# pinellolab/GRAFIMO

Hardware: AMD Instinct MI355X
Metric: scored haplotype k-mers/sec (higher is better)
Workload: dtype int32

## Files before the change

grafimo_amd/csrc/gfm_score_kernels.hpp:

```cpp
#pragma once

#include "gfm_common.hpp"

namespace {

constexpr int kWave = 64;
constexpr int kThreads = 1024;
constexpr int kWavesPerWG = kThreads / kWave;
constexpr unsigned kPoison = 0xFFFFu;
constexpr int kMaxLdsBytes = 160 * 1024;
constexpr int kWGsPerCU = 1;
constexpr int kReserveCUs = 4;
constexpr int kHitQueue = 64;

constexpr int kWorkspaces = GFM_WORKSPACE_RING;
constexpr int kCtlSlots = 2 * GFM_WORKSPACE_RING;
constexpr int kCtlAhead = GFM_WORKSPACE_RING;
struct HitCtl {
    unsigned long long mid[kCtlSlots];
    unsigned long long snap[kCtlSlots];
};
constexpr int kResidPerWG = kWavesPerWG * kHitQueue;

__device__ inline void hitq_push(long long *hitq, int &qn, bool hit, long long entry, int lane,
                                 const unsigned long long *hit_count, unsigned long long *mid,
                                 long long *hit_rows, long long hit_cap)
{
    const unsigned long long mask = __builtin_amdgcn_ballot_w64(hit);
    if (!mask) return;
    const int nh = __popcll(mask);
    if (qn + nh > kHitQueue) {
        unsigned long long base = 0;
        if (lane == 0) base = (hit_count ? *hit_count : 0ull) + atomicAdd(mid, (unsigned long long)qn);
        base = __shfl(base, 0);
        for (int i = lane; i < qn; i += kWave)
            if ((long long)(base + i) < hit_cap) hit_rows[base + i] = hitq[i];
        qn = 0;
    }
    if (hit) hitq[qn + __popcll(mask & ((1ull << lane) - 1ull))] = entry;
    qn += nh;
}

template <int WAVES>
__device__ inline void hitq_finish(const long long *hitq, int qn, int *wq_n ,
                                   int wave, int lane, int tid, long long *resid, int *resid_n)
{
    if (lane == 0) wq_n[wave] = qn;
    __syncthreads();
    int base = 0, tot = 0;
#pragma unroll
    for (int w = 0; w < WAVES; ++w) {
        if (w < wave) base += wq_n[w];
        tot += wq_n[w];
    }
    long long *slab = resid + (size_t)blockIdx.x * kResidPerWG;
    for (int i = lane; i < qn; i += kWave) slab[base + i] = hitq[i];
    if (tid == 0) resid_n[blockIdx.x] = tot;
}

constexpr int kSpillCopies = 16;

struct MotifArgs {
    const uint16_t *tab;
    int lo, nb, min_val;
    int use_hist;
    int spill_lo;
    int spill_n;
    unsigned *spill;
    int cutoff;
    int slot;
    int *scores;
    unsigned *partials;
    long long *hit_rows;
    long long hit_cap;
    const unsigned long long *hit_count;
    HitCtl *ctl;
    long long *resid;
    int *resid_n;
};
template <int MM> struct ScoreArgs {
    MotifArgs m[MM];
    int store_through;
};

typedef __attribute__((address_space(3))) const unsigned lds_cu32;
typedef __attribute__((address_space(3))) const uint16_t lds_cu16;
typedef __attribute__((address_space(3))) const unsigned long long lds_cu64;
__device__ inline unsigned lds_offset(const void *p)
{
    return (unsigned)(size_t)(__attribute__((address_space(3))) const char *)p;
}

constexpr int kSlabsPerGroup = 16;
constexpr int kPostJobs = 3;
struct PostJob {
    const unsigned *partials;
    unsigned long long *hist64;
    unsigned *spill;
    const long long *resid;
    const int *resid_n;
    HitCtl *ctl;
    long long *hit_rows;
    unsigned long long *hit_count;
    long long hit_cap;
    int nslabs, nb, lo, min_val, bin_blocks, hist_blocks, spill_lo, spill_n, spill_blocks, hit_slabs, par, total;
};
struct PostJobs { PostJob j[kPostJobs]; };

__device__ inline void
post_body(const unsigned *__restrict__ partials, int nslabs, int nb, int lo, int min_val,
          unsigned long long *__restrict__ hist64, int bin_blocks, int hist_blocks,
          unsigned *__restrict__ spill, int spill_lo, int spill_n, int spill_blocks,
          const long long *__restrict__ resid, const int *__restrict__ resid_n, int hit_slabs,
          HitCtl *__restrict__ ctl, int par, long long *__restrict__ hit_rows, long long hit_cap,
          unsigned long long *__restrict__ hit_count)
{
    const int tid = threadIdx.x;
    if (blockIdx.x == 0 && tid == 0 && hit_slabs == 0 && ctl) ctl->mid[(par + kCtlAhead) % kCtlSlots] = 0ull;
    if ((int)blockIdx.x < hist_blocks) {
        const int bx = blockIdx.x % bin_blocks, by = blockIdx.x / bin_blocks;
        const int b = bx * 256 + tid;
        if (b > nb) return;
        const int g0 = by * kSlabsPerGroup;
        const int g1 = min(g0 + kSlabsPerGroup, nslabs);
        unsigned long long s = 0;
        const size_t stride = (size_t)(nb + 1);
#pragma unroll 8
        for (int g = g0; g < g1; ++g) s += __builtin_nontemporal_load(&partials[g * stride + b]);
        if (s) atomicAdd(&hist64[b == nb ? min_val : lo + b], s);
        return;
    }
    if ((int)blockIdx.x < hist_blocks + spill_blocks) {
        const int b = ((int)blockIdx.x - hist_blocks) * 256 + tid;
        if (b < spill_n) {
            unsigned long long v = 0;
#pragma unroll
            for (int c = 0; c < kSpillCopies; ++c) {
                const unsigned x = spill[(size_t)c * (size_t)spill_n + b];
                if (x) {
                    v += x;
                    spill[(size_t)c * (size_t)spill_n + b] = 0u;
                }
            }
            if (v) atomicAdd(&hist64[spill_lo + b], v);
        }
        return;
    }
    __shared__ int part[256];
    __shared__ int part_all[256];
    const int g = blockIdx.x - hist_blocks - spill_blocks;
    int s = 0, sa = 0;
    for (int k = tid; k < hit_slabs; k += 256) {
        const int v = resid_n[k];
        sa += v;
        if (k < g) s += v;
    }
    part[tid] = s;
    part_all[tid] = sa;
    __syncthreads();
    for (int d = 128; d > 0; d >>= 1) {
        if (tid < d) { part[tid] += part[tid + d]; part_all[tid] += part_all[tid + d]; }
        __syncthreads();
    }
    const unsigned long long start = ctl->snap[par] + ctl->mid[par];
    const unsigned long long base = start + (unsigned long long)part[0];
    const int cnt = resid_n[g];
    const long long *slab = resid + (size_t)g * kResidPerWG;
    for (int i = tid; i < cnt; i += 256)
        if ((long long)(base + i) < hit_cap) __builtin_nontemporal_store(__builtin_nontemporal_load(&slab[i]), &hit_rows[base + i]);
    if (g == 0 && tid == 0) {
        *hit_count = start + (unsigned long long)part_all[0];
        ctl->mid[(par + kCtlAhead) % kCtlSlots] = 0ull;
    }
}

__global__ void __launch_bounds__(256) post_kernel(const PostJobs jobs)
{
    const PostJob &q = jobs.j[blockIdx.y];
    if ((int)blockIdx.x >= q.total) return;
    post_body(q.partials, q.nslabs, q.nb, q.lo, q.min_val, q.hist64, q.bin_blocks, q.hist_blocks, q.spill, q.spill_lo,
              q.spill_n, q.spill_blocks, q.resid, q.resid_n, q.hit_slabs, q.ctl, q.par, q.hit_rows, q.hit_cap,
              q.hit_count);
}

constexpr int kSelThreads = 256;
__global__ void __launch_bounds__(kSelThreads)
select_hits_kernel(const int *__restrict__ scores, long long n, const int *__restrict__ cutoff_ptr,
                   long long row_base, long long *__restrict__ hit_rows, long long hit_cap,
                   const unsigned long long *__restrict__ hit_count, HitCtl *__restrict__ ctl,
                   int par, long long *__restrict__ resid, int *__restrict__ resid_n,
                   const unsigned long long *__restrict__ gate_count, long long gate_cap)
{
    __shared__ long long hq[kSelThreads / kWave][kHitQueue];
    __shared__ int wq_n[kSelThreads / kWave];
    const int cutoff = *cutoff_ptr;
    const int tid = threadIdx.x, lane = tid & 63, wave = tid >> 6;
    long long *hitq = hq[wave];
    int qn = 0;
    if (gate_count) {
        if ((long long)*gate_count <= gate_cap) {
            if (tid == 0) {
                resid_n[blockIdx.x] = 0;
                if (blockIdx.x == 0) ctl->snap[par] = hit_count ? *hit_count : 0ull;
            }
            return;
        }
        hit_count = nullptr;
    }
    if (blockIdx.x == 0 && tid == 0) ctl->snap[par] = hit_count ? *hit_count : 0ull;
    const long long nthreads = (long long)gridDim.x * blockDim.x;
    const long long n4 = (n + 3) >> 2;
    const long long iters = (n4 + nthreads - 1) / nthreads;
    const long long t0 = (long long)blockIdx.x * blockDim.x + tid;
    for (long long it = 0; it < iters; ++it) {
        const long long i = t0 + it * nthreads;
        int sc[4] = {INT32_MIN, INT32_MIN, INT32_MIN, INT32_MIN};
        if (i * 4 + 4 <= n) {
            const int4 v = reinterpret_cast<const int4 *>(scores)[i];
            sc[0] = v.x; sc[1] = v.y; sc[2] = v.z; sc[3] = v.w;
        } else {
            for (int j = 0; j < 4; ++j)
                if (i * 4 + j < n) sc[j] = scores[i * 4 + j];
        }
#pragma unroll
        for (int j = 0; j < 4; ++j)
            hitq_push(hitq, qn, sc[j] >= cutoff,
                      ((row_base + i * 4 + j) << GFM_HIT_SCORE_BITS) | (long long)sc[j], lane,
                      hit_count, &ctl->mid[par], hit_rows, hit_cap);
    }
    hitq_finish<kSelThreads / kWave>(hitq, qn, wq_n, wave, lane, tid, resid, resid_n);
}

constexpr int kFilterPerThread = 16;
constexpr int kFilterPerBlock = kSelThreads * kFilterPerThread;
__global__ void __launch_bounds__(kSelThreads)
filter_hits_kernel(const long long *__restrict__ cand, const unsigned long long *__restrict__ cand_count,
                   long long cand_cap, const int *__restrict__ cutoff_ptr, long long *__restrict__ hit_rows,
                   long long hit_cap, unsigned long long *__restrict__ hit_count)
{
    __shared__ int wave_tot[kSelThreads / kWave];
    __shared__ unsigned long long block_base;
    const int cutoff = *cutoff_ptr;
    const int tid = threadIdx.x, lane = tid & 63, wave = tid >> 6;
    const unsigned long long have = *cand_count;
    if ((long long)have > cand_cap) {
        if (blockIdx.x == 0 && tid == 0) *hit_count = have;
        return;
    }
    const long long n = (long long)have;
    const long long first = (long long)blockIdx.x * kFilterPerBlock;
    if (first >= n) return;
    long long e[kFilterPerThread];
    int mine = 0;
#pragma unroll
    for (int j = 0; j < kFilterPerThread; ++j) {
        const long long i = first + (long long)j * kSelThreads + tid;
        e[j] = i < n ? cand[i] : -1ll;
        const bool keep = i < n && (int)(e[j] & ((1ll << GFM_HIT_SCORE_BITS) - 1)) >= cutoff;
        if (!keep) e[j] = -1ll;
        mine += keep ? 1 : 0;
    }
    int incl = mine;
#pragma unroll
    for (int d = 1; d < kWave; d <<= 1) {
        const int v = __shfl_up(incl, d);
        if (lane >= d) incl += v;
    }
    if (lane == kWave - 1) wave_tot[wave] = incl;
    __syncthreads();
    int before = 0, total = 0;
#pragma unroll
    for (int w = 0; w < kSelThreads / kWave; ++w) {
        if (w < wave) before += wave_tot[w];
        total += wave_tot[w];
    }
    if (tid == 0) block_base = total ? atomicAdd(hit_count, (unsigned long long)total) : 0ull;
    __syncthreads();
    unsigned long long at = block_base + (unsigned long long)(before + incl - mine);
#pragma unroll
    for (int j = 0; j < kFilterPerThread; ++j)
        if (e[j] >= 0) {
// ... 7 lines not shown
```

grafimo_amd/csrc/gfm_stats_kernels.hpp:

```cpp
#pragma once

#include "gfm_common.hpp"

namespace {

struct DpJob {
    long long sm;
    long long cum;
    long long bg;
    int W, L, lo, hi;
    double *buf;
    double *pmf;
    double *ptable;
};

constexpr int kDpThreads = 1024;

__global__ void __launch_bounds__(kDpThreads)
pvalue_dp_kernel(const DpJob *__restrict__ jobs, const int *__restrict__ ints, const double *__restrict__ dbls)
{
    const DpJob job = jobs[blockIdx.x];
    const int W = job.W, L = job.L;
    const int *__restrict__ sm = ints + job.sm;
    const int *__restrict__ cum_lo = ints + job.cum;
// ... 128 lines not shown
    unsigned long long a = 0, t = 0;
    for (int b = tid; b < nblk; b += kQThreads) {
        const unsigned long long v = ws->blk_cnt[b];
        t += v;
        if (b > blk) a += v;
    }
    const unsigned long long n = block_sum_u64(t, sh) + ws->n_rows_N;
    const unsigned long long above_blocks = block_sum_u64(a, sh);
    const double nd = (double)n;
    const int j = lo + blk * kQThreads + tid;
    const bool ok = j <= hi;
    const unsigned long long h = ok ? hist[j] : 0ull;
    unsigned long long cs = h;
#pragma unroll
    for (int d = 1; d < kWave; d <<= 1) {
        const unsigned long long v = __shfl_down(cs, d);
        if (lane + d < kWave) cs += v;
    }
    if (lane == 0) sh[wave] = cs;
    __syncthreads();
    unsigned long long waves_above = 0;
#pragma unroll
    for (int w = 0; w < kQThreads / kWave; ++w)
        if (w > wave) waves_above += sh[w];
    const unsigned long long c_ge = cs + waves_above + above_blocks;
    const double raw = h ? ptable[j] / ((double)c_ge / nd) : INFINITY;
    if (ok) raw_out[j] = raw;
    double m = raw;
#pragma unroll
    for (int d = 32; d > 0; d >>= 1) m = fmin(m, __shfl_down(m, d));
    if (lane == 0) shm[wave] = m;
    __syncthreads();
    if (tid == 0) {
        double bm = INFINITY;
        for (int w = 0; w < kQThreads / kWave; ++w) bm = fmin(bm, shm[w]);
        ws->blk_min[blk] = bm;
    }
}

__device__ inline void
q_final_body(const unsigned long long *hist, const double *__restrict__ ptable, int L, int lo,
             int hi, int min_val, double threshold, int on_qvalue, const QWork *__restrict__ ws,
             double *qtable, int *__restrict__ cutoff_out, unsigned long long *__restrict__ nrows_out,
             unsigned long long *__restrict__ clear, int nblk)
{
    __shared__ unsigned long long sh[kQThreads / kWave];
    __shared__ double shm[kQThreads / kWave];
    __shared__ int first_s;
    const int tid = threadIdx.x, lane = tid & 63, wave = tid >> 6;
    const int blk = blockIdx.x;
    if (tid == 0) first_s = L;
    unsigned long long t = 0;
    double below = INFINITY, all = INFINITY;
    for (int b = tid; b < nblk; b += kQThreads) {
        t += ws->blk_cnt[b];
        const double v = ws->blk_min[b];
        all = fmin(all, v);
        if (b < blk) below = fmin(below, v);
    }
    const unsigned long long n_rows_N = ws->n_rows_N;
    const unsigned long long n = block_sum_u64(t, sh) + n_rows_N;
    const double nd = (double)n;
#pragma unroll
    for (int d = 32; d > 0; d >>= 1) {
        below = fmin(below, __shfl_down(below, d));
        all = fmin(all, __shfl_down(all, d));
    }
    __shared__ double shb[kQThreads / kWave], sha[kQThreads / kWave];
    if (lane == 0) { shb[wave] = below; sha[wave] = all; }
    __syncthreads();
    below = INFINITY; all = INFINITY;
#pragma unroll
    for (int w = 0; w < kQThreads / kWave; ++w) { below = fmin(below, shb[w]); all = fmin(all, sha[w]); }
    const double base = n_rows_N ? ptable[min_val] / (nd / nd) : INFINITY;
    const int j = lo + blk * kQThreads + tid;
    const bool ok = j <= hi;
    double ms = ok ? qtable[j] : INFINITY;
#pragma unroll
    for (int d = 1; d < kWave; d <<= 1) {
        const double v = __shfl_up(ms, d);
        if (lane >= d) ms = fmin(ms, v);
    }
    if (lane == kWave - 1) shm[wave] = ms;
    __syncthreads();
    double waves_below = INFINITY;
#pragma unroll
    for (int w = 0; w < kQThreads / kWave; ++w)
        if (w < wave) waves_below = fmin(waves_below, shm[w]);
    const double q = fmin(fmin(fmin(ms, waves_below), fmin(below, base)), 1.0);
    if (ok) {
        qtable[j] = q;
        const double val = on_qvalue ? q : ptable[j];
        if (val < threshold) atomicMin(&first_s, j);
        if (clear) clear[j] = 0ull;
    }
    const int gtid = blk * kQThreads + tid, gsz = nblk * kQThreads;
    const double q_above = fmin(fmin(base, all), 1.0);
    for (int jj = gtid; jj < lo; jj += gsz) qtable[jj] = fmin(base, 1.0);
    for (int jj = hi + 1 + gtid; jj < L; jj += gsz) qtable[jj] = q_above;
    __syncthreads();
    if (tid == 0) {
        if (cutoff_out && first_s < L) atomicMin(cutoff_out, first_s);
        if (blk == 0) {
            if (nrows_out) *nrows_out = n;
            const bool n_outside = min_val < lo || min_val > hi;
            if (clear && n_outside) clear[min_val] = 0ull;
        }
    }
}

constexpr int kQJobs = 8;
struct QJob {
    const unsigned long long *hist;
    const double *ptable;
    QWork *ws;
    double *qtable;
    int *cutoff;
    unsigned long long *nrows;
    unsigned long long *clear;
    int L, lo, hi, min_val, nblk;
};
struct QJobs {
    QJob j[kQJobs];
    double threshold;
    int on_qvalue;
};

__global__ void __launch_bounds__(kQThreads) q_count_kernel(const QJobs jobs)
{
    const QJob &q = jobs.j[blockIdx.y];
    if ((int)blockIdx.x >= q.nblk) return;
    q_count_body(q.hist, q.L, q.lo, q.hi, q.min_val, q.ws, q.cutoff);
}

__global__ void __launch_bounds__(kQThreads) q_raw_kernel(const QJobs jobs)
{
    const QJob &q = jobs.j[blockIdx.y];
    if ((int)blockIdx.x >= q.nblk) return;
    q_raw_body(q.hist, q.ptable, q.lo, q.hi, q.ws, q.qtable, q.nblk);
}

__global__ void __launch_bounds__(kQThreads) q_final_kernel(const QJobs jobs)
{
    const QJob &q = jobs.j[blockIdx.y];
    if ((int)blockIdx.x >= q.nblk) return;
    q_final_body(q.hist, q.ptable, q.L, q.lo, q.hi, q.min_val, jobs.threshold, jobs.on_qvalue, q.ws, q.qtable,
                 q.cutoff, q.nrows, q.clear, q.nblk);
}

constexpr int kQ1Threads = 512;
constexpr int kQ1K = 16;
constexpr int kQ1Bins = kQ1Threads * kQ1K;
constexpr int kQ1Waves = kQ1Threads / kWave;

__global__ void __launch_bounds__(kQ1Threads) q_table_kernel(const QJobs jobs)
{
    const QJob &q = jobs.j[blockIdx.x];
    const unsigned long long *hist = q.hist;
    const double *__restrict__ ptable = q.ptable;
    double *qtable = q.qtable;
    unsigned long long *clear = q.clear;
    const int L = q.L, lo = q.lo, hi = q.hi, min_val = q.min_val;
    __shared__ unsigned long long sh_cnt[kQ1Waves];
    __shared__ double sh_min[kQ1Waves];
    __shared__ unsigned long long sh_n_rows_N;
    __shared__ int first_s;
    const int tid = threadIdx.x, lane = tid & (kWave - 1), wave = tid >> 6;
    const int j0 = lo + tid * kQ1K;
    const bool n_outside = min_val < lo || min_val > hi;
    if (tid == 0) {
        sh_n_rows_N = n_outside ? hist[min_val] : 0ull;
        first_s = L;
    }
    unsigned long long c[kQ1K];
    double p[kQ1K];
    unsigned occ = 0;
#pragma unroll
    for (int k = 0; k < kQ1K; ++k) c[k] = j0 + k <= hi ? hist[j0 + k] : 0ull;
#pragma unroll
    for (int k = 0; k < kQ1K; ++k) p[k] = j0 + k <= hi ? ptable[j0 + k] : 0.0;
    const double p_min_val = ptable[min_val];
    unsigned long long run = 0;
#pragma unroll
    for (int k = kQ1K - 1; k >= 0; --k) {
        occ |= (c[k] != 0ull ? 1u : 0u) << k;
        run += c[k];
        c[k] = run;
    }
    unsigned long long cs = run;
#pragma unroll
    for (int d = 1; d < kWave; d <<= 1) {
        const unsigned long long v = __shfl_down(cs, d);
        if (lane + d < kWave) cs += v;
    }
    if (lane == 0) sh_cnt[wave] = cs;
    __syncthreads();
    unsigned long long above = cs - run, total = 0;
#pragma unroll
    for (int w = 0; w < kQ1Waves; ++w) {
        const unsigned long long v = sh_cnt[w];
        total += v;
        if (w > wave) above += v;
    }
    const unsigned long long n_rows_N = sh_n_rows_N;
    const unsigned long long n = total + n_rows_N;
    const double nd = (double)n;
    double r[kQ1K];
    double m = INFINITY;
    unsigned p_below = 0;
#pragma unroll
    for (int k = 0; k < kQ1K; ++k) {
        double raw = INFINITY;
        if ((occ >> k) & 1u) raw = p[k] / ((double)(c[k] + above) / nd);
        p_below |= (p[k] < jobs.threshold ? 1u : 0u) << k;
        m = fmin(m, raw);
        r[k] = m;
    }
    double ms = m;
#pragma unroll
    for (int d = 1; d < kWave; d <<= 1) {
        const double v = __shfl_up(ms, d);
        if (lane >= d) ms = fmin(ms, v);
    }
    if (lane == kWave - 1) sh_min[wave] = ms;
    double below = __shfl_up(ms, 1);
    if (lane == 0) below = INFINITY;
    __syncthreads();
    double all = INFINITY;
#pragma unroll
    for (int w = 0; w < kQ1Waves; ++w) {
        const double v = sh_min[w];
        all = fmin(all, v);
        if (w < wave) below = fmin(below, v);
    }
    const double base = n_rows_N ? p_min_val / (nd / nd) : INFINITY;
    below = fmin(below, base);
    int first = L;
#pragma unroll
    for (int k = kQ1K - 1; k >= 0; --k) {
        const int j = j0 + k;
        if (j <= hi) {
            const double qv = fmin(fmin(r[k], below), 1.0);
            qtable[j] = qv;
            if (jobs.on_qvalue ? qv < jobs.threshold : ((p_below >> k) & 1u) != 0) first = j;
            if (clear) clear[j] = 0ull;
        }
    }
    if (first < L) atomicMin(&first_s, first);
    const double q_above = fmin(fmin(base, all), 1.0);
    for (int jj = tid; jj < lo; jj += kQ1Threads) qtable[jj] = fmin(base, 1.0);
    for (int jj = hi + 1 + tid; jj < L; jj += kQ1Threads) qtable[jj] = q_above;
    __syncthreads();
    if (tid == 0) {
        if (q.cutoff) *q.cutoff = first_s;
        if (q.nrows) *q.nrows = n;
        if (clear && n_outside) clear[min_val] = 0ull;
    }
}

}
```

grafimo_amd/csrc/grafimo_hip.hip:

```cpp

#include <hip/hip_runtime.h>

#include <algorithm>
#include <atomic>
#include <cmath>
#include <cstdarg>
#include <cstdint>
#include <cstdio>
#include <cstdlib>
#include <cstring>
#include <new>
#include <string>
#include <vector>

#include "grafimo_hip.h"

#define GFM_API extern "C" __attribute__((visibility("default")))

#include "gfm_hit_sort.hpp"
#include "gfm_common.hpp"
#include "gfm_score_kernels.hpp"
#include "gfm_quad_launch.hpp"
#include "gfm_stats_kernels.hpp"

struct gfm_motif {
    int W = 0, L = 0, min_val = 0, scale = 1, ndw = 0;
    double offset = 0.0;
    int lo = 0, hi = 0, nb = 0;
    int hlo = 0, hnb = 0;
    int q_waves = kWavesPerWG;
    int part_nb = 0;
    struct Window { int bins, lo; double mass; };
    std::vector<Window> windows;
    int device = 0;
    int n_cu = 256;
    int max_slabs = 0;
    int sel_slabs = 0;
    int reserve_cus = kReserveCUs;
    size_t lds_bytes = 0;
    std::vector<int64_t> sm;
    double bg[4] = {0, 0, 0, 0};
    std::vector<double> h_ptable;
    unsigned char *d_slab = nullptr;
    uint16_t *d_tab = nullptr;
    unsigned *d_ftab = nullptr;
    double *d_pmf = nullptr;
    double *d_ptable = nullptr;
    unsigned *d_partials[kWorkspaces] = {};
    unsigned *d_spill[kWorkspaces] = {};
    long long *d_resid[kWorkspaces] = {};
    int *d_resid_n[kWorkspaces] = {};
    QWork *d_qwork = nullptr;
    double *d_qscratch = nullptr;
    hipStream_t q_stream[kQStreams] = {};
    int q_streams_used = 0;
    unsigned long long q_last_use[kQStreams] = {}, q_calls = 0;
    hipEvent_t ev_selected = nullptr;
    hipStream_t sel_last_stream = nullptr;
    bool sel_valid = false;
    HitCtl *d_ctl = nullptr;
    unsigned call_no = 0;
    hipStream_t last_st = nullptr, last_tail = nullptr;
    unsigned same_pair_run = 0;
    hipEvent_t ev_scored[kWorkspaces] = {};
    hipStream_t launch_st[2] = {};
    hipEvent_t launch_last[2] = {};
    hipEvent_t ev_join[kWorkspaces] = {};
    unsigned quiet = 0;
    bool overlap_on = true;
    unsigned long long overlapped = 0;
    hipEvent_t ev_posted[kWorkspaces] = {};
    bool posted_valid[kWorkspaces] = {};
    long long *d_sel_resid = nullptr;
    int *d_sel_resid_n = nullptr;
    HitCtl *d_sel_ctl = nullptr;
    unsigned sel_call_no = 0;
    std::vector<hipEvent_t> ev0, ev1;
    int ev_next = 0, ev_used = 0, ev_every = 1;
    unsigned ev_calls = 0;
    std::vector<hipEvent_t> tev0, tev1;
    int ev_last = -1;
    int tail_pending = -1;
    std::vector<int> tail_order;
};

namespace {

int ensure_device()
{
    int n = 0;
    hipError_t e = hipGetDeviceCount(&n);
    if (e != hipSuccess || n <= 0) {
        (void)hipGetLastError();
        return fail(GFM_ERR_NODEVICE, "no HIP device available (%s)",
                    e == hipSuccess ? "device count is 0" : hipGetErrorString(e));
    }
    return GFM_OK;
}

void cumulative_windows(const int64_t *sm, int W, std::vector<int> &lo, std::vector<int> &hi)
{
    lo.resize(W);
    hi.resize(W);
    long long l = 0, h = 0;
    for (int j = 0; j < W; ++j) {
        int64_t mn = sm[j], mx = sm[j];
        for (int nuc = 1; nuc < 4; ++nuc) {
            mn = std::min(mn, sm[nuc * W + j]);
            mx = std::max(mx, sm[nuc * W + j]);
        }
        l += mn;
        h += mx;
        lo[j] = (int)l;
        hi[j] = (int)h;
    }
}

int validate_matrix(const int64_t *sm, int W, int i)
{
    if (!sm) return fail(GFM_ERR_INVALID, "motif %d: score matrix is NULL", i);
    if (W < 1 || W > GFM_MAX_WIDTH)
        return fail(GFM_ERR_INVALID, "motif %d: motif width %d outside [1, %d]", i, W, GFM_MAX_WIDTH);
    for (int k = 0; k < 4 * W; ++k)
        if (sm[k] < 0 || sm[k] > kRange)
            return fail(GFM_ERR_INVALID, "motif %d: scaled score %lld outside [0, %d]", i, (long long)sm[k], kRange);
    return GFM_OK;
}

size_t align256(size_t bytes) { return (bytes + 255) & ~(size_t)255; }

struct DpPack {
    std::vector<DpJob> jobs;
    std::vector<int> ints;
    std::vector<double> dbls;

    DpJob &add(const int64_t *sm, int W, const double *bg)
    {
        std::vector<int> lo, hi;
        cumulative_windows(sm, W, lo, hi);
        DpJob j{};
        j.sm = (long long)ints.size();
        for (int i = 0; i < 4 * W; ++i) ints.push_back((int)sm[i]);
        j.cum = (long long)ints.size();
        ints.insert(ints.end(), lo.begin(), lo.end());
        ints.insert(ints.end(), hi.begin(), hi.end());
        j.bg = (long long)dbls.size();
        dbls.insert(dbls.end(), bg, bg + 4);
        j.W = W;
        j.L = kRange * W + 1;
        j.lo = lo[W - 1];
        j.hi = hi[W - 1];
        jobs.push_back(j);
        return jobs.back();
    }
    size_t ints_at() const { return align256(sizeof(DpJob) * jobs.size()); }
    size_t dbls_at() const { return ints_at() + align256(sizeof(int) * ints.size()); }
    size_t bytes() const { return dbls_at() + sizeof(double) * dbls.size(); }
    std::vector<unsigned char> image() const
    {
        std::vector<unsigned char> img(bytes(), 0);
        std::memcpy(img.data(), jobs.data(), sizeof(DpJob) * jobs.size());
        std::memcpy(img.data() + ints_at(), ints.data(), sizeof(int) * ints.size());
        std::memcpy(img.data() + dbls_at(), dbls.data(), sizeof(double) * dbls.size());
        return img;
    }
    int launch(const unsigned char *d, int n_dp, bool tails, hipStream_t st) const
    {
        const DpJob *d_jobs = reinterpret_cast<const DpJob *>(d);
        if (n_dp > 0) {
            hipLaunchKernelGGL(pvalue_dp_kernel, dim3((unsigned)n_dp), dim3(kDpThreads), 0, st, d_jobs,
                               reinterpret_cast<const int *>(d + ints_at()),
                               reinterpret_cast<const double *>(d + dbls_at()));
            HIP_TRY(hipGetLastError());
        }
        if (tails && !jobs.empty()) {
            hipLaunchKernelGGL(ptable_kernel, dim3((unsigned)jobs.size()), dim3(kScanThreads), 0, st, d_jobs);
            HIP_TRY(hipGetLastError());
        }
        return GFM_OK;
    }
};

int dispatch_quad(int W, int mm, gfm_motif *timer, const uint8_t *d_kmers, long long n, long long row_base,
                  const void *args, size_t lds, int nslabs, int waves, hipStream_t st, bool prepare_only,
                  hipEvent_t *done = nullptr)
{
    if (W < 1 || W > GFM_MAX_WIDTH) return fail(GFM_ERR_INVALID, "unsupported width %d", W);
    if (mm < 1 || mm > 3 || (mm > 1 && W > kQuadMaxBatchWidth))
        return fail(GFM_ERR_INVALID, "no kernel for %d motifs of width %d in one launch", mm, W);
    hipEvent_t e0 = nullptr, e1 = done ? *done : nullptr;
    if (!prepare_only && timer && !timer->ev0.empty() && (timer->ev_calls++ % (unsigned)timer->ev_every) == 0) {
        e0 = timer->ev0[timer->ev_next];
        e1 = timer->ev1[timer->ev_next];
        if (done) *done = e1;
        timer->ev_last = timer->ev_next;
        timer->ev_next = (timer->ev_next + 1) % (int)timer->ev0.size();
        timer->ev_used = std::min(timer->ev_used + 1, (int)timer->ev0.size());
    } else if (timer) {
        timer->ev_last = -1;
    }
    typedef int (*launch_fn)(int, const uint8_t *, long long, long long, const void *, size_t, int, int, void *, int,
                             void *, void *);
    static const launch_fn table[3][4] = {
        {gfm_quad_launch_g0_m1, gfm_quad_launch_g1_m1, gfm_quad_launch_g2_m1, gfm_quad_launch_g3_m1},
        {gfm_quad_launch_g0_m2, gfm_quad_launch_g1_m2, nullptr, nullptr},
        {gfm_quad_launch_g0_m3, gfm_quad_launch_g1_m3, nullptr, nullptr}};
    return table[mm - 1][(W - 1) / 16](W, d_kmers, n, row_base, args, lds, nslabs, waves, st, prepare_only ? 1 : 0, e0, e1);
}

constexpr long long kStoreThroughMaxBytes = 96ll << 20;
int score_store_through(long long n, int mm)
{
#ifdef GFM_LAB
    if (const char *e = std::getenv("GRAFIMO_STORE_POLICY")) {
        if (!std::strcmp(e, "through")) return 1;
        if (!std::strcmp(e, "stream")) return 0;
    }
#endif
    return n * 4ll * mm <= kStoreThroughMaxBytes ? 1 : 0;
}

size_t quad_fixed_lds(int W, int waves, int mm = 1)
{
    return (size_t)quad_tab_bytes(W, mm) + (size_t)waves * (size_t)quad_strip_stride(W, mm);
}

gfm_motif::Window best_window(gfm_motif *m, int bins)
{
    if (bins >= m->nb) return {m->nb, m->lo, 1.0};
    for (const auto &w : m->windows)
        if (w.bins == bins) return w;
    gfm_motif::Window best{bins, m->lo, -1.0};
    for (int a = m->lo; a + bins - 1 <= m->hi; ++a) {
        const int e = a + bins;
        const double mass = m->h_ptable[a] - (e < m->L ? m->h_ptable[e] : 0.0);
        if (mass > best.mass) { best.mass = mass; best.lo = a; }
    }
    m->windows.push_back(best);
    return best;
}

PostJob post_job(gfm_motif *m, const unsigned *partials, int hist_slabs, unsigned long long *d_hist,
                 int win_lo, int win_nb, unsigned *spill, const long long *resid, const int *resid_n, int hit_slabs,
                 HitCtl *ctl, int ctl_slot, long long *d_hit_rows, long long cap, unsigned long long *d_hit_count)
{
    PostJob q{};
    q.bin_blocks = (win_nb + 1 + 255) / 256;
    const int groups = (hist_slabs + kSlabsPerGroup - 1) / kSlabsPerGroup;
    q.hist_blocks = d_hist ? q.bin_blocks * groups : 0;
    q.spill_blocks = (d_hist && spill && win_nb < m->nb) ? (m->nb + 255) / 256 : 0;
    q.total = q.hist_blocks + q.spill_blocks + hit_slabs;
    q.partials = partials; q.hist64 = d_hist; q.spill = spill; q.resid = resid; q.resid_n = resid_n; q.ctl = ctl;
    q.hit_rows = d_hit_rows; q.hit_count = d_hit_count; q.hit_cap = cap;
    q.nslabs = hist_slabs; q.nb = win_nb; q.lo = win_lo; q.min_val = m->min_val;
    q.spill_lo = m->lo; q.spill_n = m->nb; q.hit_slabs = hit_slabs; q.par = ctl_slot;
    return q;
}

int launch_posts(const PostJob *jobs, int count, hipStream_t st)
{
    PostJobs all{};
    int live = 0, max_total = 0;
    for (int k = 0; k < count; ++k) {
        const PostJob &q = jobs[k];
        if (q.total == 0) {
            if (q.ctl)
                HIP_TRY(hipMemsetAsync(&q.ctl->mid[(q.par + kCtlAhead) % kCtlSlots], 0, sizeof(unsigned long long), st));
            continue;
        }
        all.j[live++] = q;
        max_total = std::max(max_total, q.total);
    }
    if (live == 0) return GFM_OK;
    hipLaunchKernelGGL(post_kernel, dim3((unsigned)max_total, (unsigned)live), dim3(256), 0, st, all);
    HIP_TRY(hipGetLastError());
    return GFM_OK;
}

int launch_post(gfm_motif *m, const unsigned *partials, int hist_slabs, unsigned long long *d_hist,
                int win_lo, int win_nb, unsigned *spill, const long long *resid, const int *resid_n, int hit_slabs, HitCtl *ctl, int ctl_slot,
                long long *d_hit_rows, long long cap, unsigned long long *d_hit_count, hipStream_t st)
{
    const PostJob q = post_job(m, partials, hist_slabs, d_hist, win_lo, win_nb, spill, resid, resid_n, hit_slabs, ctl,
                               ctl_slot, d_hit_rows, cap, d_hit_count);
    return launch_posts(&q, 1, st);
}

int join_launch_streams(gfm_motif *m, hipStream_t st)
{
    for (int i = 0; i < 2; ++i) {
        if (!m->launch_last[i]) continue;
        HIP_TRY(hipStreamWaitEvent(st, m->launch_last[i], 0));
        m->launch_last[i] = nullptr;
    }
    return GFM_OK;
}

__global__ void launch_stream_warm_kernel() {}

int ensure_launch_streams(gfm_motif *m)
{
    for (int i = 0; i < 2; ++i) {
        if (m->launch_st[i]) continue;
        HIP_TRY(hipStreamCreateWithFlags(&m->launch_st[i], hipStreamNonBlocking));
        hipLaunchKernelGGL(launch_stream_warm_kernel, dim3(1), dim3(kWave), 0, m->launch_st[i]);
        HIP_TRY(hipGetLastError());
    }
    for (int i = 0; i < kWorkspaces; ++i)
        if (!m->ev_join[i]) HIP_TRY(hipEventCreateWithFlags(&m->ev_join[i], hipEventDisableTiming));
    return GFM_OK;
}

int caller_stream_idle(gfm_motif *m, hipStream_t st, bool *idle)
{
    *idle = false;
    if (m->quiet) {
        --m->quiet;
        return GFM_OK;
    }
    const hipError_t q = hipStreamQuery(st);
    if (q != hipSuccess) {
        (void)hipGetLastError();
        if (q != hipErrorNotReady) HIP_TRY(q);
        m->quiet = 3;
        return GFM_OK;
    }
    *idle = true;
    return GFM_OK;
}

void fill_motif_args(MotifArgs &a, gfm_motif *m, int ws, int slot, int use_hist, int win_lo, int win_nb,
                     int cutoff,
                     int *d_scores, long long *d_hit_rows, long long cap,
                     const unsigned long long *d_hit_count_or_null)
{
    a.tab = m->d_tab;
    a.lo = win_lo;
    a.nb = win_nb;
    a.min_val = m->min_val;
    a.use_hist = use_hist;
    a.spill_lo = m->lo;
    a.spill_n = m->nb;
    a.spill = m->d_spill[ws];
    a.cutoff = cutoff;
    a.slot = slot;
    a.scores = d_scores;
    a.partials = m->d_partials[ws];
    a.hit_rows = d_hit_rows;
    a.hit_cap = cap;
    a.hit_count = d_hit_count_or_null;
    a.ctl = m->d_ctl;
    a.resid = m->d_resid[ws];
    a.resid_n = m->d_resid_n[ws];
}

bool plan_group(const gfm_motif_t *motifs, int n_left, const bool *with_hist, int *mm_out, int *waves_out,
                int *win_lo, int *win_nb)
{
    constexpr double kMinWindowMass = 0.999;
    const int W = motifs[0]->W;
    int mm = std::min(W <= kQuadMaxBatchWidth ? 3 : 1, n_left);
    int waves = kWavesPerWG;
    bool found = false;
    for (; mm >= 1 && !found; --mm) {
        for (int pass = mm > 1 ? 0 : 1; pass < 2 && !found; ++pass) {
            for (waves = kWavesPerWG; waves >= kWavesPerWG / 2 && !found; waves /= 2) {
                const long long spare = (long long)kMaxLdsBytes - (long long)quad_fixed_lds(W, waves, mm);
                long long room = spare / (long long)sizeof(unsigned);
                bool open[3] = {false, false, false};
                int users = 0;
                for (int k = 0; k < mm; ++k) {
                    win_nb[k] = 0;
                    win_lo[k] = motifs[k]->lo;
                    open[k] = with_hist[k];
                    users += open[k];
                }
                bool ok = spare >= 0 && (room > 0 || users == 0);
                for (bool again = true; ok && again && users > 0;) {
                    again = false;
                    const long long share = room / users - 1;
                    for (int k = 0; k < mm; ++k)
                        if (open[k] && motifs[k]->nb <= share) {
                            win_nb[k] = motifs[k]->nb;
                            room -= win_nb[k] + 1;
                            open[k] = false;
                            --users;
                            again = true;
                        }
                }
                if (ok && users > 0) {
                    const long long share = room / users - 1;
                    if (pass == 0 || share < 256) ok = false;
                    for (int k = 0; ok && k < mm; ++k)
                        if (open[k]) {
                            const gfm_motif::Window w = best_window(motifs[k], (int)share);
                            win_nb[k] = w.bins;
                            win_lo[k] = w.lo;
                            if ((mm > 1 || waves > kWavesPerWG / 2) && w.mass < kMinWindowMass) ok = false;
                        }
                }
                found = ok;
                if (found) break;
            }
            if (found) break;
        }
        if (found) break;
    }
    *mm_out = mm;
    *waves_out = waves;
    return found;
}

}

extern "C" __attribute__((visibility("hidden"))) void gfm_set_error_(const char *msg) { g_err = msg ? msg : ""; }

extern "C" __attribute__((visibility("hidden"))) int gfm_motif_view_(gfm_motif_t m, int max_bins, int small_bins, const int64_t **sm,
                                                                     int *W, int *min_val, int *L, int *win_lo, int *win_nb,
                                                                     int *device, int *n_cu, const unsigned **d_ftab)
{
    if (!m) return fail(GFM_ERR_INVALID, "motif is NULL");
    gfm_motif::Window w = best_window(m, std::max(1, std::min(max_bins, m->nb)));
    if (small_bins > 0 && small_bins < w.bins) {
        const gfm_motif::Window ws = best_window(m, small_bins);
#ifndef GFM_GRAPH_SMALL_MASS
#define GFM_GRAPH_SMALL_MASS 0.9
#endif
#ifdef GFM_LAB
        static const double need = [] { const char *e = std::getenv("GRAFIMO_FUSED_SMALL_MASS"); return e ? atof(e) : GFM_GRAPH_SMALL_MASS; }();
#else
        constexpr double need = GFM_GRAPH_SMALL_MASS;
#endif
        if (ws.mass >= need) w = ws;
    }
    *sm = m->sm.data();
    *W = m->W;
    *min_val = m->min_val;
    *L = m->L;
// ... 411 lines not shown
    if (hi) *hi = m->hi;
    return GFM_OK;
}

GFM_API int gfm_motif_tables(gfm_motif_t m, double *h_pmf, double *h_ptable)
{
    if (!m) return fail(GFM_ERR_INVALID, "motif is NULL");
    if (h_pmf) HIP_TRY(hipMemcpy(h_pmf, m->d_pmf, sizeof(double) * (size_t)m->L, hipMemcpyDeviceToHost));
    if (h_ptable) std::memcpy(h_ptable, m->h_ptable.data(), sizeof(double) * (size_t)m->L);
    return GFM_OK;
}

GFM_API int gfm_motif_pvalue_cutoff(gfm_motif_t m, double threshold, int32_t *cutoff)
{
    if (!m || !cutoff) return fail(GFM_ERR_INVALID, "NULL argument");
    int a = 0, b = m->L;
    while (a < b) {
        const int mid = (a + b) / 2;
        if (m->h_ptable[mid] < threshold) b = mid; else a = mid + 1;
    }
    *cutoff = a;
    return GFM_OK;
}

GFM_API int gfm_motif_annotate(gfm_motif_t m, const int32_t *scores, int64_t n, double *lo_out,
                               double *p_out)
{
    if (!m || (!scores && n)) return fail(GFM_ERR_INVALID, "NULL argument");
    for (int64_t i = 0; i < n; ++i) {
        const int s = scores[i];
        if (s < 0 || s >= m->L) return fail(GFM_ERR_INVALID, "score %d outside the table", s);
        if (lo_out) lo_out[i] = ((double)s / (double)m->scale) + ((double)m->W * m->offset);
        if (p_out) p_out[i] = m->h_ptable[s];
    }
    return GFM_OK;
}

GFM_API int gfm_score_kmers(gfm_motif_t m, const uint8_t *d_kmers, int64_t n, int32_t *d_scores,
                            uint64_t *d_hist, int32_t select_cutoff, int64_t row_base,
                            int64_t *d_hit_rows, int64_t hit_capacity, uint64_t *d_hit_count,
                            uint32_t flags, void *stream, void *tail_stream)
{
    if (!m) return fail(GFM_ERR_INVALID, "motif is NULL");
    if (n < 0) return fail(GFM_ERR_INVALID, "negative row count");
    hipStream_t st = static_cast<hipStream_t>(stream);
    hipStream_t tail = tail_stream ? static_cast<hipStream_t>(tail_stream) : st;
    const bool split = tail != st;
    if (n == 0) {
        if ((flags & GFM_FLAG_RESET_HITS) && d_hit_count) {
            if (split) {
                const int rcj = join_launch_streams(m, st);
                if (rcj) return rcj;
                HIP_TRY(hipEventRecord(m->ev_scored[0], st));
                HIP_TRY(hipStreamWaitEvent(tail, m->ev_scored[0], 0));
            }
            HIP_TRY(hipMemsetAsync(d_hit_count, 0, sizeof(uint64_t), tail));
        }
        return GFM_OK;
    }
    if (!d_kmers) return fail(GFM_ERR_INVALID, "NULL device buffer");
    {
        int dev = -1;
        HIP_TRY(hipGetDevice(&dev));
        if (dev != m->device)
            return fail(GFM_ERR_INVALID, "the motif lives on device %d, the current device is %d", m->device, dev);
    }
    if ((reinterpret_cast<uintptr_t>(d_kmers) & 15u) != 0)
        return fail(GFM_ERR_INVALID, "d_kmers must be 16-byte aligned");
    if ((reinterpret_cast<uintptr_t>(d_scores) & 3u) != 0)
        return fail(GFM_ERR_INVALID, "d_scores must be 4-byte aligned");
    if (!d_scores && !d_hist && select_cutoff == GFM_NO_SELECT)
        return fail(GFM_ERR_INVALID, "nothing to do: no scores, no histogram, no selection");
    if (n > (int64_t)kQuadRows * 0x7fffff00ll)
        return fail(GFM_ERR_INVALID, "too many rows for one launch (split the batch)");
    const bool select = select_cutoff != GFM_NO_SELECT;
    if (select && (!d_hit_rows || !d_hit_count))
        return fail(GFM_ERR_INVALID, "selection requested without hit buffers");
    const int use_hist = d_hist ? 1 : 0;
    const long long nchunks = (n + kQuadRows - 1) / kQuadRows;
    const long long want = (nchunks + m->q_waves - 1) / m->q_waves;
    const int avail = split ? std::max(1, m->max_slabs - m->reserve_cus * (m->max_slabs / m->n_cu)) : m->max_slabs;
    int nslabs = (int)std::min<long long>(want, avail);
    if (want > avail) {
        long long best_cap = -1;
        for (int g = avail; g >= std::max(1, avail - avail / 8); --g) {
            const long long per_turn = (long long)g * m->q_waves;
            const long long cap = (nchunks + per_turn - 1) / per_turn * per_turn;
            if (best_cap < 0 || cap < best_cap) { best_cap = cap; nslabs = g; }
        }
    }

    const unsigned k = m->call_no++;
    const int ws = (int)(k % (unsigned)kWorkspaces), slot = (int)(k % (unsigned)kCtlSlots);
    const int ws_prev = (int)((k + kWorkspaces - 1) % (unsigned)kWorkspaces);
    const bool reset = (flags & GFM_FLAG_RESET_HITS) != 0;
    const bool same_owner = st == m->last_st && tail == m->last_tail;
    const bool caller_orders = (flags & GFM_FLAG_CALLER_ORDERS_REUSE) && same_owner && m->same_pair_run >= (unsigned)kWorkspaces;
    const bool orders_next = (flags & GFM_FLAG_CALLER_ORDERS_REUSE) && same_owner && m->same_pair_run + 1 == (unsigned)kWorkspaces;
    m->same_pair_run = same_owner ? m->same_pair_run + 1 : 1;
    m->last_st = st;
    m->last_tail = tail;
    bool overlap = false, idle = false;
    if ((flags & GFM_FLAG_OVERLAP_LAUNCHES) && split && m->overlap_on && !(select && !reset) &&
        (caller_orders || orders_next)) {
        int rco = ensure_launch_streams(m);
        if (!rco && caller_orders) {
            overlap = true;
            rco = caller_stream_idle(m, st, &idle);
        }
        if (rco) return rco;
    }
    hipStream_t kst = overlap ? m->launch_st[k & 1u] : st;
    if (overlap && !idle) {
        HIP_TRY(hipEventRecord(m->ev_join[ws], st));
        HIP_TRY(hipStreamWaitEvent(kst, m->ev_join[ws], 0));
    }
    if (overlap && want > avail) nslabs = avail;
#ifdef GFM_LAB
    if (const char *e = std::getenv("GRAFIMO_SCORE_GRID")) {
        const int g = atoi(e);
        if (want > avail && g >= 1 && g <= m->max_slabs) nslabs = g;
    }
#endif
    if (!overlap) {
        const int rcj = join_launch_streams(m, st);
        if (rcj) return rcj;
    }
    if (m->posted_valid[ws] && !caller_orders)
        HIP_TRY(hipStreamWaitEvent(st, m->ev_posted[ws], 0));
    if (split && select && !reset && m->posted_valid[ws_prev])
        HIP_TRY(hipStreamWaitEvent(st, m->ev_posted[ws_prev], 0));
    ScoreArgs<1> args{};
    args.store_through = d_scores ? score_store_through(n, 1) : 2;
    fill_motif_args(args.m[0], m, ws, slot, use_hist, m->hlo, m->hnb, select_cutoff, d_scores,
                    reinterpret_cast<long long *>(d_hit_rows), hit_capacity,
                    reset ? nullptr : reinterpret_cast<unsigned long long *>(d_hit_count));
    hipEvent_t scored = split ? m->ev_scored[ws] : nullptr;
    int rc = dispatch_quad(m->W, 1, m, d_kmers, n, row_base, &args, m->lds_bytes, nslabs, m->q_waves, kst, false,
                           split ? &scored : nullptr);
    if (rc) return rc;
    if (overlap) {
        m->launch_last[k & 1u] = scored;
        if (idle) ++m->overlapped;
    }
    if (split) HIP_TRY(hipStreamWaitEvent(tail, scored, 0));
    m->tail_pending = -1;
    if (split && m->ev_last >= 0 && !m->tev0.empty()) {
        HIP_TRY(hipEventRecord(m->tev0[m->ev_last], tail));
        m->tail_pending = m->ev_last;
    }
    rc = launch_post(m, m->d_partials[ws], nslabs, reinterpret_cast<unsigned long long *>(d_hist),
                     m->hlo, m->hnb, m->d_spill[ws], m->d_resid[ws], m->d_resid_n[ws], select ? nslabs : 0, m->d_ctl, slot,
                     reinterpret_cast<long long *>(d_hit_rows), hit_capacity,
                     reinterpret_cast<unsigned long long *>(d_hit_count), tail);
    if (rc) return rc;
    if (split) {
        HIP_TRY(hipEventRecord(m->ev_posted[ws], tail));
        m->posted_valid[ws] = true;
    } else {
        m->posted_valid[ws] = false;
    }
    return GFM_OK;
}

GFM_API int gfm_score_kmers_multi(const gfm_motif_t *motifs, int n_motifs, const uint8_t *d_kmers,
                                  int64_t n, int32_t *const *d_scores, uint64_t *const *d_hist,
                                  const int32_t *select_cutoffs, int64_t row_base,
                                  int64_t *const *d_hit_rows, const int64_t *hit_capacity,
                                  uint64_t *const *d_hit_count, uint32_t flags, void *stream)
{
    if (!motifs || n_motifs < 1) return fail(GFM_ERR_INVALID, "NULL argument");
    if (n < 0) return fail(GFM_ERR_INVALID, "negative row count");
    hipStream_t st = static_cast<hipStream_t>(stream);
    const bool reset = (flags & GFM_FLAG_RESET_HITS) != 0;
    bool no_scores = d_scores == nullptr;
    if (d_scores) {
        int n_null = 0;
        for (int i = 0; i < n_motifs; ++i) n_null += d_scores[i] ? 0 : 1;
        if (n_null != 0 && n_null != n_motifs) return fail(GFM_ERR_INVALID, "d_scores: every entry or none (scores are stored for all motifs of a call or for none)");
        no_scores = n_null == n_motifs;
    }
    for (int i = 0; i < n_motifs; ++i) {
        if (!motifs[i]) return fail(GFM_ERR_INVALID, "motif %d is NULL", i);
        if (motifs[i]->W != motifs[0]->W)
            return fail(GFM_ERR_INVALID, "motifs of one batched launch must share their width (%d vs %d)",
                        motifs[i]->W, motifs[0]->W);
        for (int j = 0; j < i; ++j)
            if (motifs[j] == motifs[i]) return fail(GFM_ERR_INVALID, "motif %d listed twice", i);
        const bool sel = select_cutoffs && select_cutoffs[i] != GFM_NO_SELECT;
        if (sel && (!d_hit_rows || !d_hit_rows[i] || !d_hit_count || !d_hit_count[i] || !hit_capacity))
            return fail(GFM_ERR_INVALID, "selection requested for motif %d without hit buffers", i);
    }
    if (n == 0) {
        if (reset && d_hit_count)
            for (int i = 0; i < n_motifs; ++i)
                if (d_hit_count[i]) HIP_TRY(hipMemsetAsync(d_hit_count[i], 0, sizeof(uint64_t), st));
        return GFM_OK;
    }
    if (!d_kmers) return fail(GFM_ERR_INVALID, "NULL device buffer");
    if ((reinterpret_cast<uintptr_t>(d_kmers) & 15u) != 0)
        return fail(GFM_ERR_INVALID, "d_kmers must be 16-byte aligned");
    if (n > (int64_t)kQuadRows * 0x7fffff00ll)
        return fail(GFM_ERR_INVALID, "too many rows for one launch (split the batch)");
    for (int i = 0; i < n_motifs && !no_scores; ++i)
        if ((reinterpret_cast<uintptr_t>(d_scores[i]) & 3u) != 0)
            return fail(GFM_ERR_INVALID, "d_scores[%d] must be 4-byte aligned", i);
    const int W = motifs[0]->W;
    const long long nchunks = (n + kQuadRows - 1) / kQuadRows;

    int i = 0;
    while (i < n_motifs) {
        int mm = 0, waves = kWavesPerWG, nb_lds[3] = {0, 0, 0};
        int win_lo[3] = {0, 0, 0}, win_nb[3] = {0, 0, 0};
        bool with_hist[3];
        for (int k = 0; k < 3; ++k) with_hist[k] = i + k < n_motifs && d_hist && d_hist[i + k];
        if (!plan_group(motifs + i, n_motifs - i, with_hist, &mm, &waves, win_lo, win_nb))
            return fail(GFM_ERR_INVALID, "no LDS left for a histogram window at width %d", W);
        for (int k = 0; k < mm; ++k) {
            if (win_nb[k] > motifs[i + k]->part_nb)
                return fail(GFM_ERR_INVALID, "internal error: histogram window larger than the workspace");
            nb_lds[k] = (d_hist && d_hist[i + k]) ? win_nb[k] + 1 : 0;
        }
        size_t lds = quad_fixed_lds(W, waves, mm);
        for (int k = 0; k < mm; ++k) lds += sizeof(unsigned) * (size_t)nb_lds[k];
        const long long want = (nchunks + waves - 1) / waves;
        int nslabs = (int)std::min<long long>(want, motifs[i]->max_slabs);
        for (int k = 1; k < mm; ++k) nslabs = std::min(nslabs, motifs[i + k]->max_slabs);
        int ws[3], slot[3], uh[3];
        ScoreArgs<1> a1{};
        ScoreArgs<2> a2{};
        ScoreArgs<3> a3{};
        a1.store_through = a2.store_through = a3.store_through = no_scores ? 2 : score_store_through(n, mm);
        for (int k = 0; k < mm; ++k) {
            gfm_motif *mo = motifs[i + k];
            const unsigned c = mo->call_no++;
            mo->same_pair_run = 0;
            mo->last_st = mo->last_tail = nullptr;
            if (const int rcj = join_launch_streams(mo, st)) return rcj;
            ws[k] = (int)(c % (unsigned)kWorkspaces);
            slot[k] = (int)(c % (unsigned)kCtlSlots);
            mo->posted_valid[ws[k]] = false;
            uh[k] = (d_hist && d_hist[i + k]) ? 1 : 0;
            const int cut = select_cutoffs ? select_cutoffs[i + k] : GFM_NO_SELECT;
            const bool sel = cut != GFM_NO_SELECT;
            MotifArgs &dst = mm == 1 ? a1.m[k] : (mm == 2 ? a2.m[k] : a3.m[k]);
            fill_motif_args(dst, mo, ws[k], slot[k], uh[k], win_lo[k], win_nb[k], cut, no_scores ? nullptr : d_scores[i + k],
                            sel ? reinterpret_cast<long long *>(d_hit_rows[i + k]) : nullptr,
                            sel ? hit_capacity[i + k] : 0,
                            (sel && !reset) ? reinterpret_cast<const unsigned long long *>(d_hit_count[i + k])
                                            : nullptr);
        }
        const void *args = mm == 1 ? static_cast<const void *>(&a1) : (mm == 2 ? static_cast<const void *>(&a2) : &a3);
        int rc = dispatch_quad(W, mm, motifs[i], d_kmers, n, row_base, args, lds, nslabs, waves, st, false);
        if (rc) return rc;
        PostJob posts[kPostJobs];
        for (int k = 0; k < mm; ++k) {
            gfm_motif *mo = motifs[i + k];
            const int cut = select_cutoffs ? select_cutoffs[i + k] : GFM_NO_SELECT;
            const bool sel = cut != GFM_NO_SELECT;
            posts[k] = post_job(mo, mo->d_partials[ws[k]], nslabs,
                                uh[k] ? reinterpret_cast<unsigned long long *>(d_hist[i + k]) : nullptr,
                                win_lo[k], win_nb[k], mo->d_spill[ws[k]], mo->d_resid[ws[k]], mo->d_resid_n[ws[k]],
                                sel ? nslabs : 0, mo->d_ctl, slot[k],
                                sel ? reinterpret_cast<long long *>(d_hit_rows[i + k]) : nullptr,
                                sel ? hit_capacity[i + k] : 0,
                                sel ? reinterpret_cast<unsigned long long *>(d_hit_count[i + k]) : nullptr);
        }
        rc = launch_posts(posts, mm, st);
        if (rc) return rc;
        i += mm;
    }
    return GFM_OK;
}

GFM_API int gfm_score_kmers_multi_plan(const gfm_motif_t *motifs, int n_motifs, const int32_t *with_hist,
                                       int32_t *group_size_out, int32_t *waves_out)
{
    if (!motifs || n_motifs < 1) return fail(GFM_ERR_INVALID, "NULL argument");
    for (int i = 0; i < n_motifs; ++i) {
        if (!motifs[i]) return fail(GFM_ERR_INVALID, "motif %d is NULL", i);
        if (motifs[i]->W != motifs[0]->W)
            return fail(GFM_ERR_INVALID, "motifs of one batched launch must share their width (%d vs %d)",
                        motifs[i]->W, motifs[0]->W);
    }
    int i = 0;
    while (i < n_motifs) {
        int mm = 0, waves = 0, win_lo[3], win_nb[3];
        bool wh[3];
        for (int k = 0; k < 3; ++k) wh[k] = i + k < n_motifs && (!with_hist || with_hist[i + k]);
        if (!plan_group(motifs + i, n_motifs - i, wh, &mm, &waves, win_lo, win_nb))
            return fail(GFM_ERR_INVALID, "no LDS left for a histogram window at width %d", motifs[0]->W);
        for (int k = 0; k < mm; ++k) {
            if (group_size_out) group_size_out[i + k] = mm;
            if (waves_out) waves_out[i + k] = waves;
        }
        i += mm;
    }
    return GFM_OK;
}

GFM_API int gfm_motif_set_overlap(gfm_motif_t m, int enabled)
{
    if (!m) return fail(GFM_ERR_INVALID, "motif is NULL");
    m->overlap_on = enabled != 0;
    return GFM_OK;
}

GFM_API int gfm_overlapped_launches(gfm_motif_t m, uint64_t *count)
{
    if (!m || !count) return fail(GFM_ERR_INVALID, "NULL argument");
    *count = m->overlapped;
    return GFM_OK;
}

// ... 367 lines not shown
```

Baseline: 249.0 billion.

## Batch partial-slab loads, coalesce q-table via LDS staging, fuse post event record

The post kernel's histogram reduction now issues all slab loads of a full group before summing, which raises memory-level parallelism. The q_table kernel now loads hist and ptable in a coalesced strided pattern and transposes them through a padded LDS buffer. It writes qtable back the same way instead of having each thread touch 16 consecutive elements. The event after the post kernel is now recorded through hipExtLaunchKernelGGL's stop-event argument instead of a separate hipEventRecord. That adds a large shared-memory array and extra barriers to q_table_kernel, and a lab-only env hook for splitting post parts.

Result: no change. 248.3 billion (-0.3%).

```diff
diff --git a/grafimo_amd/csrc/gfm_score_kernels.hpp b/grafimo_amd/csrc/gfm_score_kernels.hpp
--- a/grafimo_amd/csrc/gfm_score_kernels.hpp
+++ b/grafimo_amd/csrc/gfm_score_kernels.hpp
@@ -125,8 +125,16 @@
         const int g1 = min(g0 + kSlabsPerGroup, nslabs);
         unsigned long long s = 0;
         const size_t stride = (size_t)(nb + 1);
+        if (g1 - g0 == kSlabsPerGroup) {
+            unsigned v[kSlabsPerGroup];
+#pragma unroll
+            for (int k = 0; k < kSlabsPerGroup; ++k) v[k] = __builtin_nontemporal_load(&partials[(g0 + k) * stride + b]);
+#pragma unroll
+            for (int k = 0; k < kSlabsPerGroup; ++k) s += v[k];
+        } else {
 #pragma unroll 8
-        for (int g = g0; g < g1; ++g) s += __builtin_nontemporal_load(&partials[g * stride + b]);
+            for (int g = g0; g < g1; ++g) s += __builtin_nontemporal_load(&partials[g * stride + b]);
+        }
         if (s) atomicAdd(&hist64[b == nb ? min_val : lo + b], s);
         return;
     }
diff --git a/grafimo_amd/csrc/gfm_stats_kernels.hpp b/grafimo_amd/csrc/gfm_stats_kernels.hpp
--- a/grafimo_amd/csrc/gfm_stats_kernels.hpp
+++ b/grafimo_amd/csrc/gfm_stats_kernels.hpp
@@ -304,6 +304,8 @@
 constexpr int kQ1K = 16;
 constexpr int kQ1Bins = kQ1Threads * kQ1K;
 constexpr int kQ1Waves = kQ1Threads / kWave;
+constexpr int kQ1Pitch = kQ1K + 1;
+__device__ inline int q1_slot(int i) { return i + i / kQ1K; }
 
 __global__ void __launch_bounds__(kQ1Threads) q_table_kernel(const QJobs jobs)
 {
@@ -313,6 +315,7 @@
     double *qtable = q.qtable;
     unsigned long long *clear = q.clear;
     const int L = q.L, lo = q.lo, hi = q.hi, min_val = q.min_val;
+    __shared__ unsigned long long stage[kQ1Threads * kQ1Pitch];
     __shared__ unsigned long long sh_cnt[kQ1Waves];
     __shared__ double sh_min[kQ1Waves];
     __shared__ unsigned long long sh_n_rows_N;
@@ -320,6 +323,19 @@
     const int tid = threadIdx.x, lane = tid & (kWave - 1), wave = tid >> 6;
     const int j0 = lo + tid * kQ1K;
     const bool n_outside = min_val < lo || min_val > hi;
+    unsigned long long cg[kQ1K];
+    double pg[kQ1K];
+#pragma unroll
+    for (int k = 0; k < kQ1K; ++k) {
+        const int j = lo + k * kQ1Threads + tid;
+        cg[k] = j <= hi ? hist[j] : 0ull;
+    }
+#pragma unroll
+    for (int k = 0; k < kQ1K; ++k) {
+        const int j = lo + k * kQ1Threads + tid;
+        pg[k] = j <= hi ? ptable[j] : 0.0;
+    }
+    const double p_min_val = ptable[min_val];
     if (tid == 0) {
         sh_n_rows_N = n_outside ? hist[min_val] : 0ull;
         first_s = L;
@@ -328,10 +344,16 @@
     double p[kQ1K];
     unsigned occ = 0;
 #pragma unroll
-    for (int k = 0; k < kQ1K; ++k) c[k] = j0 + k <= hi ? hist[j0 + k] : 0ull;
-#pragma unroll
-    for (int k = 0; k < kQ1K; ++k) p[k] = j0 + k <= hi ? ptable[j0 + k] : 0.0;
-    const double p_min_val = ptable[min_val];
+    for (int k = 0; k < kQ1K; ++k) stage[q1_slot(k * kQ1Threads + tid)] = cg[k];
+    __syncthreads();
+#pragma unroll
+    for (int k = 0; k < kQ1K; ++k) c[k] = stage[tid * kQ1Pitch + k];
+    __syncthreads();
+#pragma unroll
+    for (int k = 0; k < kQ1K; ++k) stage[q1_slot(k * kQ1Threads + tid)] = (unsigned long long)__double_as_longlong(pg[k]);
+    __syncthreads();
+#pragma unroll
+    for (int k = 0; k < kQ1K; ++k) p[k] = __longlong_as_double((long long)stage[tid * kQ1Pitch + k]);
     unsigned long long run = 0;
 #pragma unroll
     for (int k = kQ1K - 1; k >= 0; --k) {
@@ -391,18 +413,23 @@
 #pragma unroll
     for (int k = kQ1K - 1; k >= 0; --k) {
         const int j = j0 + k;
-        if (j <= hi) {
-            const double qv = fmin(fmin(r[k], below), 1.0);
-            qtable[j] = qv;
-            if (jobs.on_qvalue ? qv < jobs.threshold : ((p_below >> k) & 1u) != 0) first = j;
-            if (clear) clear[j] = 0ull;
-        }
+        const double qv = fmin(fmin(r[k], below), 1.0);
+        stage[tid * kQ1Pitch + k] = (unsigned long long)__double_as_longlong(qv);
+        if (j <= hi && (jobs.on_qvalue ? qv < jobs.threshold : ((p_below >> k) & 1u) != 0)) first = j;
     }
     if (first < L) atomicMin(&first_s, first);
     const double q_above = fmin(fmin(base, all), 1.0);
     for (int jj = tid; jj < lo; jj += kQ1Threads) qtable[jj] = fmin(base, 1.0);
     for (int jj = hi + 1 + tid; jj < L; jj += kQ1Threads) qtable[jj] = q_above;
     __syncthreads();
+#pragma unroll
+    for (int k = 0; k < kQ1K; ++k) {
+        const int i = k * kQ1Threads + tid, j = lo + i;
+        if (j <= hi) {
+            qtable[j] = __longlong_as_double((long long)stage[q1_slot(i)]);
+            if (clear) clear[j] = 0ull;
+        }
+    }
     if (tid == 0) {
         if (q.cutoff) *q.cutoff = first_s;
         if (q.nrows) *q.nrows = n;
diff --git a/grafimo_amd/csrc/grafimo_hip.hip b/grafimo_amd/csrc/grafimo_hip.hip
--- a/grafimo_amd/csrc/grafimo_hip.hip
+++ b/grafimo_amd/csrc/grafimo_hip.hip
@@ -1,5 +1,6 @@
 
 #include <hip/hip_runtime.h>
+#include <hip/hip_ext.h>
 
 #include <algorithm>
 #include <atomic>
@@ -257,12 +258,19 @@
     return q;
 }
 
-int launch_posts(const PostJob *jobs, int count, hipStream_t st)
+int launch_posts(const PostJob *jobs, int count, hipStream_t st, hipEvent_t done = nullptr)
 {
     PostJobs all{};
     int live = 0, max_total = 0;
+#ifdef GFM_LAB
+    const char *parts = std::getenv("GRAFIMO_POST_PARTS");
+#endif
     for (int k = 0; k < count; ++k) {
-        const PostJob &q = jobs[k];
+        PostJob q = jobs[k];
+#ifdef GFM_LAB
+        if (parts && !std::strcmp(parts, "hist")) q.total = q.hist_blocks + q.spill_blocks;
+        if (parts && !std::strcmp(parts, "hits")) { q.hist_blocks = q.spill_blocks = 0; q.total = q.hit_slabs; }
+#endif
         if (q.total == 0) {
             if (q.ctl)
                 HIP_TRY(hipMemsetAsync(&q.ctl->mid[(q.par + kCtlAhead) % kCtlSlots], 0, sizeof(unsigned long long), st));
@@ -271,19 +279,26 @@
         all.j[live++] = q;
         max_total = std::max(max_total, q.total);
     }
-    if (live == 0) return GFM_OK;
-    hipLaunchKernelGGL(post_kernel, dim3((unsigned)max_total, (unsigned)live), dim3(256), 0, st, all);
+    if (live == 0) {
+        if (done) HIP_TRY(hipEventRecord(done, st));
+        return GFM_OK;
+    }
+    const dim3 grid((unsigned)max_total, (unsigned)live);
+    if (done)
+        hipExtLaunchKernelGGL(post_kernel, grid, dim3(256), 0, st, nullptr, done, 0, all);
+    else
+        hipLaunchKernelGGL(post_kernel, grid, dim3(256), 0, st, all);
     HIP_TRY(hipGetLastError());
     return GFM_OK;
 }
 
 int launch_post(gfm_motif *m, const unsigned *partials, int hist_slabs, unsigned long long *d_hist,
                 int win_lo, int win_nb, unsigned *spill, const long long *resid, const int *resid_n, int hit_slabs, HitCtl *ctl, int ctl_slot,
-                long long *d_hit_rows, long long cap, unsigned long long *d_hit_count, hipStream_t st)
+                long long *d_hit_rows, long long cap, unsigned long long *d_hit_count, hipStream_t st, hipEvent_t done = nullptr)
 {
     const PostJob q = post_job(m, partials, hist_slabs, d_hist, win_lo, win_nb, spill, resid, resid_n, hit_slabs, ctl,
                                ctl_slot, d_hit_rows, cap, d_hit_count);
-    return launch_posts(&q, 1, st);
+    return launch_posts(&q, 1, st, done);
 }
 
 int join_launch_streams(gfm_motif *m, hipStream_t st)
@@ -1001,14 +1016,9 @@
     rc = launch_post(m, m->d_partials[ws], nslabs, reinterpret_cast<unsigned long long *>(d_hist),
                      m->hlo, m->hnb, m->d_spill[ws], m->d_resid[ws], m->d_resid_n[ws], select ? nslabs : 0, m->d_ctl, slot,
                      reinterpret_cast<long long *>(d_hit_rows), hit_capacity,
-                     reinterpret_cast<unsigned long long *>(d_hit_count), tail);
+                     reinterpret_cast<unsigned long long *>(d_hit_count), tail, split ? m->ev_posted[ws] : nullptr);
     if (rc) return rc;
-    if (split) {
-        HIP_TRY(hipEventRecord(m->ev_posted[ws], tail));
-        m->posted_valid[ws] = true;
-    } else {
-        m->posted_valid[ws] = false;
-    }
+    m->posted_valid[ws] = split;
     return GFM_OK;
 }
 
```
